# atenpas/agile_grasp

Hardware: AMD Instinct MI355X
Metric: grasp hypotheses/sec on 300k-pt cloud @2000 samples (higher is better)
Workload: dtype f64

## Files before the change

### agile_grasp_amd/csrc/taubin.hip

```cpp
#include "agh_internal.h"

#include <cstring>
#include <utility>

#include "taubin_eigen.h"

namespace agh
{

constexpr int kSortBins = 256;
constexpr int kChunk = 56;

template <int CAP>
__device__ __forceinline__ void taubin_moments_sample(const int s, GridView gv, const float* __restrict__ xyz, int64_t stride,
  const int32_t* __restrict__ samples, int S, float r2f, double rpad, int first_class, double* __restrict__ sums,
  int32_t* __restrict__ nt, int32_t* __restrict__ status, float4* __restrict__ nbr, int64_t nbr_stride, int debug_stop,
  int n_points, int32_t* __restrict__ zero_flags, int32_t* __restrict__ scloud, long long* __restrict__ dbg,
  int32_t* __restrict__ ovf_out)
{
#ifdef AGH_DEBUG_HOOKS
#define AGH_MSTAMP(i) do { if (dbg && threadIdx.x == 0) dbg[(int64_t) blockIdx.x * 8 + (i)] = wall_clock64(); } while (0)
  long long mt_prod = 0, mt_cons = 0, mt_wait = 0, mt_last = 0;
#define AGH_MLAP(acc) do { if (dbg) { const long long now_ = wall_clock64(); acc += now_ - mt_last; mt_last = now_; } } while (0)
#else
#define AGH_MSTAMP(i) do { } while (0)
#define AGH_MLAP(acc) do { } while (0)
#endif
  AGH_MSTAMP(0);
  constexpr int kSortBytes = CAP * 8 + CAP * 2 + (kSortBins + 1) * 4 + kSortBins * 4;
  constexpr int kTS = kChunk + 2;
  constexpr int kTermBytes = kNumSums * kTS * 8;
  constexpr int kScratch = ((kSortBytes > kTermBytes ? kSortBytes : kTermBytes) + 15) & ~15;
  __shared__ float4 stage[CAP];
  __shared__ unsigned short slot[CAP];
  __shared__ __attribute__((aligned(16))) unsigned char scratch[kScratch];
  __shared__ RowTable rt;
  __shared__ int count;
  __shared__ int wsum[4];
  unsigned long long* key = reinterpret_cast<unsigned long long*>(scratch);
  unsigned short* perm = reinterpret_cast<unsigned short*>(scratch + CAP * 8);
  int* hist = reinterpret_cast<int*>(scratch + CAP * 8 + CAP * 2);
  int* fillc = hist + (kSortBins + 1);
  double* termbuf = reinterpret_cast<double*>(scratch);

  const int tid = threadIdx.x, lane = tid & 63, wave = tid >> 6;
  if (zero_flags && blockIdx.x == 0 && tid < 8)
    zero_flags[tid] = 0;
  if (!first_class && status[s] != kStatusOverflow)
    return;
  const int n_pts = n_points >= 0 ? n_points : gv.cloud_off[gv.n_clouds];
  if (samples[s] < 0 || samples[s] >= n_pts)
  {
    if (threadIdx.x == 0)
    {
      status[s] = samples[s] == kSampleSkip ? kStatusSkipped : kStatusBadIndex;
      nt[s] = 0;
    }
    return;
  }
  const float* qp = xyz + (int64_t) samples[s] * stride;
  const float qx = qp[0], qy = qp[1], qz = qp[2];
  {
    const int cloud = cloud_of_point(gv, samples[s]);
    gv = grid_of_cloud(gv, cloud);
    if (first_class && tid == 0)
      scloud[s] = cloud;
  }
  if (!(isfinite(qx) && isfinite(qy) && isfinite(qz)))
  {
    if (tid == 0)
    {
      status[s] = kStatusOk;
      nt[s] = 0;
    }
    return;
  }
  if (tid == 0)
    count = 0;
  for (int k = tid; k < kSortBins; k += 256)
  {
    hist[k] = 0;
    fillc[k] = 0;
  }
  build_rows(gv, qx, qy, qz, rpad, rt);
  if (rt.bad)
  {
    if (tid == 0)
    {
      status[s] = kStatusRows;
      nt[s] = 0;
    }
    return;
  }
  AGH_MSTAMP(1);
  const float binscale = (float) kSortBins / r2f;
  {
    FlatRows flat;
    flat.init(rt, lane);
    const int nseg = flat.segments();
    auto seg_load = [&](int j, int& r0, float4& p0, float4& p1, bool& h0, bool& h1) {
      int a0, a1;
      flat.locate(j, r0, lane, a0, a1, h0, h1);
      p0 = gv.sorted[h0 ? a0 : 0];
      p1 = gv.sorted[h1 ? a1 : 0];
    };
    auto take2 = [&](const float4& p0, bool h0, const float4& p1, bool h1) {
      const float d0 = flann_d2(qx, qy, qz, p0.x, p0.y, p0.z), d1 = flann_d2(qx, qy, qz, p1.x, p1.y, p1.z);
      const bool s0 = h0 & (d0 < r2f), s1 = h1 & (d1 < r2f);
      const unsigned long long m0 = __ballot(s0), m1 = __ballot(s1);
      if (m0 | m1)
      {
        const int c0 = __popcll(m0);
        int base = 0;
        if (lane == 0)
          base = atomicAdd(&count, c0 + __popcll(m1));
        base = __builtin_amdgcn_readfirstlane(base);
        const unsigned long long below = (1ull << lane) - 1ull;
        const int k0 = base + __popcll(m0 & below), k1 = base + c0 + __popcll(m1 & below);
        if (s0 && k0 < CAP)
        {
          stage[k0] = p0;
          key[k0] = ((unsigned long long) __float_as_uint(d0) << 32) | (unsigned long long) __float_as_uint(p0.w);
          atomicAdd(&hist[min(kSortBins - 1, (int) (d0 * binscale))], 1);
        }
        if (s1 && k1 < CAP)
        {
          stage[k1] = p1;
          key[k1] = ((unsigned long long) __float_as_uint(d1) << 32) | (unsigned long long) __float_as_uint(p1.w);
          atomicAdd(&hist[min(kSortBins - 1, (int) (d1 * binscale))], 1);
        }
      }
    };
    int cur_j = wave, r0 = 0;
    float4 p0, p1;
    bool h0, h1;
    seg_load(cur_j, r0, p0, p1, h0, h1);
    while (cur_j < nseg)
    {
      float4 q0, q1;
      bool g0, g1;
      seg_load(cur_j + 4, r0, q0, q1, g0, g1);
      take2(p0, h0, p1, h1);
      cur_j += 4;
      p0 = q0;
      p1 = q1;
      h0 = g0;
      h1 = g1;
    }
  }
  __syncthreads();
  const int n = count;
  if (n > CAP)
  {
    if (tid == 0)
    {
      status[s] = kStatusOverflow;
      nt[s] = n;
      if (ovf_out)
        ovf_out[1 + atomicAdd(&ovf_out[0], 1)] = s;
    }
    return;
  }
  AGH_MSTAMP(2);
  if (debug_stop == 1)
    return;
  {
    const int lane_ = tid & 63, w_ = tid >> 6;
    const int v = hist[tid];
    const int inc = wave_incl_scan_i32(v);
    if (lane_ == 63)
      wsum[w_] = inc;
    __syncthreads();
    int base = 0;
    for (int k = 0; k < w_; k++)
      base += wsum[k];
    hist[tid] = base + inc - v;
    if (tid == 0)
      hist[kSortBins] = n;
    __syncthreads();
  }
  {
    constexpr int kPerThread = CAP <= 1152 ? (CAP + 255) / 256 : 1;
    for (int k0 = tid; k0 < n; k0 += 256 * kPerThread)
    {
      int bb[kPerThread], pos[kPerThread];
#pragma unroll
      for (int u = 0; u < kPerThread; u++)
      {
        const int k = k0 + 256 * u;
        const float d2 = __uint_as_float((unsigned) (key[k < n ? k : k0] >> 32));
        bb[u] = min(kSortBins - 1, (int) (d2 * binscale));
      }
#pragma unroll
      for (int u = 0; u < kPerThread; u++)
        pos[u] = (k0 + 256 * u < n) ? hist[bb[u]] + atomicAdd(&fillc[bb[u]], 1) : 0;
#pragma unroll
      for (int u = 0; u < kPerThread; u++)
        if (k0 + 256 * u < n)
          perm[pos[u]] = (unsigned short) (k0 + 256 * u);
    }
  }
  __syncthreads();
  for (int g = tid; g < n; g += 256)
  {
    const int k = perm[g];
    const unsigned long long mine = key[k];
    const float d2 = __uint_as_float((unsigned) (mine >> 32));
    const int b = min(kSortBins - 1, (int) (d2 * binscale));
    const int bs = hist[b], be = hist[b + 1];
    int rank = bs;
    for (int g2 = bs; g2 < be; g2 += 4)
    {
      unsigned short pk[4];
#pragma unroll
      for (int u = 0; u < 4; u++)
        pk[u] = perm[min(g2 + u, be - 1)];
      unsigned long long kk[4];
#pragma unroll
      for (int u = 0; u < 4; u++)
        kk[u] = key[pk[u]];
#pragma unroll
      for (int u = 0; u < 4; u++)
        rank += (g2 + u < be && kk[u] < mine) ? 1 : 0;
    }
    slot[rank] = (unsigned short) k;
  }
  __syncthreads();
  if (debug_stop == 2)
    return;
  AGH_MSTAMP(3);
  {
    constexpr int kPerThread = CAP <= 1152 ? (CAP + 255) / 256 : 1;
    for (int i0 = tid; i0 < n; i0 += 256 * kPerThread)
    {
      unsigned short sl[kPerThread];
#pragma unroll
      for (int u = 0; u < kPerThread; u++)
        sl[u] = slot[min(i0 + 256 * u, n > 0 ? n - 1 : 0)];
      float4 pv[kPerThread];
#pragma unroll
      for (int u = 0; u < kPerThread; u++)
        pv[u] = stage[sl[u]];
#pragma unroll
      for (int u = 0; u < kPerThread; u++)
        if (i0 + 256 * u < n)
          nbr[(int64_t) s * nbr_stride + i0 + 256 * u] = pv[u];
    }
  }
  double acc = 0.0;
#ifdef AGH_DEBUG_HOOKS
  mt_last = wall_clock64();
#endif
  const int n_last = n > 0 ? n - 1 : 0;
  float4 p_next = stage[slot[min(lane, n_last)]];
  for (int c0 = 0; c0 < n; c0 += kChunk)
  {
    const int rows = min(kChunk, n - c0);
    const float4 p = p_next;
    p_next = stage[slot[min(c0 + kChunk + lane, n_last)]];
    if (lane < rows && wave < 2)
    {
      const double x = (double) p.x, y = (double) p.y, z = (double) p.z;
      const double x2 = x * x, y2 = y * y, z2 = z * z;
      const double xy = x * y, yz = y * z, xz = x * z;
      double* t = &termbuf[lane];
      if (wave == 0)
      {
        t[0 * kTS] = x2 * x2;
        t[1 * kTS] = x2 * y2;
        t[2 * kTS] = x2 * z2;
        t[3 * kTS] = x2 * xy;
        t[4 * kTS] = x2 * yz;
        t[5 * kTS] = x2 * xz;
        t[6 * kTS] = x2 * x;
        t[7 * kTS] = x2 * y;
        t[8 * kTS] = x2 * z;
        t[9 * kTS] = x2;
        t[10 * kTS] = y2 * y2;
        t[11 * kTS] = y2 * z2;
        t[12 * kTS] = y2 * xy;
        t[13 * kTS] = y2 * yz;
        t[14 * kTS] = y2 * xz;
        t[15 * kTS] = y2 * x;
        t[16 * kTS] = y2 * y;
        t[17 * kTS] = y2 * z;
        t[18 * kTS] = y2;
      }
      else
      {
        t[19 * kTS] = z2 * z2;
        t[20 * kTS] = z2 * xy;
        t[21 * kTS] = z2 * yz;
        t[22 * kTS] = z2 * xz;
        t[23 * kTS] = z2 * x;
        t[24 * kTS] = z2 * y;
        t[25 * kTS] = z2 * z;
        t[26 * kTS] = z2;
        t[27 * kTS] = x * yz;
        t[28 * kTS] = xy;
        t[29 * kTS] = yz;
        t[30 * kTS] = xz;
        t[31 * kTS] = x;
        t[32 * kTS] = y;
        t[33 * kTS] = z;
        t[34 * kTS] = x2 + y2;
        t[35 * kTS] = y2 + z2;
        t[36 * kTS] = x2 + z2;
      }
    }
    __syncthreads();
    AGH_MLAP(mt_prod);
    if (wave == 0 && lane < kNumSums && rows == kChunk)
    {
      double2 va[kChunk / 2];
#pragma unroll
      for (int u = 0; u < kChunk / 2; u++)
        va[u] = reinterpret_cast<const double2*>(termbuf + lane * kTS)[u];
#pragma unroll
      for (int u = 0; u < kChunk / 2; u++)
      {
        acc += va[u].x;
        acc += va[u].y;
      }
    }
    else if (wave == 0 && lane < kNumSums)
    {
      int k = 0;
      for (; k + 8 <= rows; k += 8)
      {
        double v_[8];
#pragma unroll
        for (int u = 0; u < 8; u++)
          v_[u] = termbuf[lane * kTS + k + u];
#pragma unroll
        for (int u = 0; u < 8; u++)
          acc += v_[u];
      }
      for (; k < rows; k++)
        acc += termbuf[lane * kTS + k];
    }
#ifdef AGH_DEBUG_HOOKS
    if (dbg && acc == 1.2345e300)
      mt_cons++;
#endif
    AGH_MLAP(mt_cons);
    __syncthreads();
    AGH_MLAP(mt_wait);
  }
  if (wave == 0 && lane < kNumSums)
    sums[(int64_t) s * kSumStride + lane] = acc;
  if (tid == 0)
  {
    nt[s] = n;
    status[s] = kStatusOk;
  }
  AGH_MSTAMP(4);
#ifdef AGH_DEBUG_HOOKS
  if (dbg && threadIdx.x == 0)
  {
    dbg[(int64_t) blockIdx.x * 8 + 5] = mt_prod;
    dbg[(int64_t) blockIdx.x * 8 + 6] = mt_cons;
    dbg[(int64_t) blockIdx.x * 8 + 7] = mt_wait;
  }
#endif
#undef AGH_MSTAMP
#undef AGH_MLAP
}

template <int CAP>
__global__ __launch_bounds__(256, CAP <= 1152 ? 4 : 1) void k_taubin_moments(GridView gv, const float* __restrict__ xyz, int64_t stride,
  const int32_t* __restrict__ samples, int S, float r2f, double rpad, int first_class, double* __restrict__ sums,
  int32_t* __restrict__ nt, int32_t* __restrict__ status, float4* __restrict__ nbr, int64_t nbr_stride, int debug_stop,
  int n_points, int32_t* __restrict__ zero_flags, int32_t* __restrict__ scloud, long long* __restrict__ dbg,
  int32_t* __restrict__ ovf_out, const int32_t* __restrict__ ovf_list)
{
  if constexpr (CAP == 4096)
  {
    const int n_items = ovf_list ? min(ovf_list[0], S) : S;
    for (int it = blockIdx.x; it < n_items; it += gridDim.x)
    {
      taubin_moments_sample<CAP>(ovf_list ? ovf_list[1 + it] : it, gv, xyz, stride, samples, S, r2f, rpad, first_class, sums, nt, status,
        nbr, nbr_stride, debug_stop, n_points, zero_flags, scloud, dbg, ovf_out);
      if (it + (int) gridDim.x < n_items)
        __syncthreads();
    }
  }
  else
    taubin_moments_sample<CAP>((int) blockIdx.x, gv, xyz, stride, samples, S, r2f, rpad, first_class, sums, nt, status, nbr, nbr_stride,
      debug_stop, n_points, zero_flags, scloud, dbg, ovf_out);
}

__global__ __launch_bounds__(256) void k_taubin_moments_huge(GridView gv, const float* __restrict__ xyz, int64_t stride,
  const int32_t* __restrict__ samples, int S, float r2f, double rpad, double* __restrict__ sums, int32_t* __restrict__ nt,
  int32_t* __restrict__ status, float4* __restrict__ nbr, int64_t nbr_stride, float4* __restrict__ pool_stage,
  unsigned long long* __restrict__ pool_key, float4* __restrict__ pool_sorted, long long* __restrict__ huge_base,
  unsigned long long* __restrict__ pool_count)
{
  constexpr int kTS = kChunk + 2;
  constexpr int kKeyTile = 2048;
  __shared__ __attribute__((aligned(16))) double termbuf[kNumSums * kTS];
  __shared__ unsigned long long ktile[kKeyTile];
  __shared__ RowTable rt;
  __shared__ int count, n_s;
  __shared__ long long base_s;
  const int s = blockIdx.x;
  const int tid = threadIdx.x, lane = tid & 63, wave = tid >> 6;
  if (tid == 0)
    huge_base[s] = -1;
  if (status[s] != kStatusOverflow)
    return;
  if (tid == 0)
    count = 0;
  const float* qp = xyz + (int64_t) samples[s] * stride;
  const float qx = qp[0], qy = qp[1], qz = qp[2];
  gv = grid_of_cloud(gv, cloud_of_point(gv, samples[s]));
  build_rows(gv, qx, qy, qz, rpad, rt);
  if (rt.bad)
    return;
  {
    int mine = 0;
    for (int j = tid; j < rt.total; j += 256)
    {
      const float4 p = gv.sorted[row_lookup(rt, j)];
      mine += flann_d2(qx, qy, qz, p.x, p.y, p.z) < r2f ? 1 : 0;
    }
    mine = wave_allsum_i32(mine);
    if (lane == 0 && mine)
      atomicAdd(&count, mine);
  }
  __syncthreads();
  if (tid == 0)
  {
    const int n0 = count;
    n_s = n0;
    const unsigned long long b0 = atomicAdd(pool_count, (unsigned long long) n0);
    base_s = b0 + (unsigned long long) n0 <= (unsigned long long) kHugeEntries ? (long long) b0 : -1;
    count = 0;
  }
  __syncthreads();
  const int n = n_s;
  const long long base = base_s;
  if (base < 0)
  {
    if (tid == 0)
      nt[s] = n;
    return;
  }
  float4* stage = pool_stage + base;
  unsigned long long* key = pool_key + base;
  for (int j = tid; j < rt.total; j += 256)
  {
    const float4 p = gv.sorted[row_lookup(rt, j)];
    const float d2 = flann_d2(qx, qy, qz, p.x, p.y, p.z);
    if (d2 < r2f)
    {
      const int k = atomicAdd(&count, 1);
      stage[k] = p;
      key[k] = ((unsigned long long) __float_as_uint(d2) << 32) | (unsigned long long) __float_as_uint(p.w);
    }
  }
  __threadfence();
  __syncthreads();
  const bool in_pool = n > nbr_stride;
  float4* const list_w = in_pool ? pool_sorted + base : nbr + (int64_t) s * nbr_stride;
  if (tid == 0)
    huge_base[s] = in_pool ? base : -1;
  for (int g0 = 0; g0 < n; g0 += 256 * 8)
  {
    constexpr int kPer = 8;
    unsigned long long mine[kPer];
    int rank[kPer];
#pragma unroll
    for (int u = 0; u < kPer; u++)
    {
      const int g = g0 + tid + 256 * u;
      mine[u] = g < n ? key[g] : ~0ull;
      rank[u] = 0;
    }
    for (int t0 = 0; t0 < n; t0 += kKeyTile)
    {
      const int tn = min(kKeyTile, n - t0);
      __syncthreads();
      for (int k = tid; k < tn; k += 256)
        ktile[k] = key[t0 + k];
      __syncthreads();
      for (int k = 0; k < tn; k++)
      {
        const unsigned long long kk = ktile[k];
#pragma unroll
        for (int u = 0; u < kPer; u++)
          rank[u] += kk < mine[u] ? 1 : 0;
      }
    }
#pragma unroll
    for (int u = 0; u < kPer; u++)
    {
      const int g = g0 + tid + 256 * u;
      if (g < n)
        list_w[rank[u]] = stage[g];
    }
  }
  __threadfence();
  __syncthreads();
  const float4* list = list_w;
  double acc = 0.0;
  for (int c0 = 0; c0 < n; c0 += kChunk)
  {
    const int rows = min(kChunk, n - c0);
    if (lane < rows && wave < 2)
    {
      const float4 p = list[c0 + lane];
      const double x = (double) p.x, y = (double) p.y, z = (double) p.z;
      const double x2 = x * x, y2 = y * y, z2 = z * z;
      const double xy = x * y, yz = y * z, xz = x * z;
      double* t = &termbuf[lane];
      if (wave == 0)
      {
        t[0 * kTS] = x2 * x2;
        t[1 * kTS] = x2 * y2;
        t[2 * kTS] = x2 * z2;
        t[3 * kTS] = x2 * xy;
        t[4 * kTS] = x2 * yz;
        t[5 * kTS] = x2 * xz;
        t[6 * kTS] = x2 * x;
        t[7 * kTS] = x2 * y;
        t[8 * kTS] = x2 * z;
        t[9 * kTS] = x2;
        t[10 * kTS] = y2 * y2;
        t[11 * kTS] = y2 * z2;
        t[12 * kTS] = y2 * xy;
        t[13 * kTS] = y2 * yz;
        t[14 * kTS] = y2 * xz;
        t[15 * kTS] = y2 * x;
        t[16 * kTS] = y2 * y;
        t[17 * kTS] = y2 * z;
        t[18 * kTS] = y2;
      }
      else
      {
        t[19 * kTS] = z2 * z2;
        t[20 * kTS] = z2 * xy;
        t[21 * kTS] = z2 * yz;
        t[22 * kTS] = z2 * xz;
        t[23 * kTS] = z2 * x;
        t[24 * kTS] = z2 * y;
        t[25 * kTS] = z2 * z;
        t[26 * kTS] = z2;
        t[27 * kTS] = x * yz;
        t[28 * kTS] = xy;
        t[29 * kTS] = yz;
        t[30 * kTS] = xz;
        t[31 * kTS] = x;
        t[32 * kTS] = y;
        t[33 * kTS] = z;
        t[34 * kTS] = x2 + y2;
        t[35 * kTS] = y2 + z2;
        t[36 * kTS] = x2 + z2;
      }
    }
    __syncthreads();
    if (wave == 0 && lane < kNumSums)
      for (int k = 0; k < rows; k++)
        acc += termbuf[lane * kTS + k];
    __syncthreads();
  }
  if (wave == 0 && lane < kNumSums)
    sums[(int64_t) s * kSumStride + lane] = acc;
  if (tid == 0)
  {
    nt[s] = n;
    status[s] = kStatusOk;
  }
}

constexpr int kOrderBins = 2048;
constexpr int kOrderMaxSamples = 4096;
__device__ __forceinline__ int order_bin(int w) { return kOrderBins - 1 - min(w >> 4, kOrderBins - 1); }

__device__ void sample_order_block(const int* __restrict__ weight, int S, int* __restrict__ order, int* hist, int* wave_tot)
{
  constexpr int kPer = 16, kT = 256;
  const int tid = threadIdx.x, lane = tid & 63, wave = tid >> 6;
  for (int b = tid; b < kOrderBins; b += kT)
    hist[b] = 0;
  __syncthreads();
  for (int base = 0; base < S; base += kT * kPer)
  {
    int bin[kPer];
#pragma unroll
    for (int u = 0; u < kPer; u++)
    {
      const int s = base + u * kT + tid;
      bin[u] = s < S ? order_bin(weight[s]) : -1;
    }
#pragma unroll
    for (int u = 0; u < kPer; u++)
      if (bin[u] >= 0)
        atomicAdd(&hist[bin[u]], 1);
  }
  __syncthreads();
  constexpr int per = kOrderBins / kT;
  int loc = 0;
  for (int k = 0; k < per; k++)
    loc += hist[tid * per + k];
  int incl = loc;
  incl = wave_incl_scan_i32(incl);
  if (lane == 63)
    wave_tot[wave] = incl;
  __syncthreads();
  int run = incl - loc;
  for (int w = 0; w < wave; w++)
    run += wave_tot[w];
  for (int k = 0; k < per; k++)
  {
    const int c = hist[tid * per + k];
    hist[tid * per + k] = run;
    run += c;
  }
  __syncthreads();
  for (int base = 0; base < S; base += kT * kPer)
  {
    int bin[kPer], pos[kPer];
#pragma unroll
    for (int u = 0; u < kPer; u++)
    {
      const int s = base + u * kT + tid;
      bin[u] = s < S ? order_bin(weight[s]) : -1;
    }
#pragma unroll
    for (int u = 0; u < kPer; u++)
      pos[u] = bin[u] >= 0 ? atomicAdd(&hist[bin[u]], 1) : 0;
#pragma unroll
    for (int u = 0; u < kPer; u++)
      if (bin[u] >= 0)
        order[pos[u]] = base + u * kT + tid;
  }
}

constexpr int kSweepBlock = 32, kSweepBlocksMax = 1024;
__device__ void sweep_order_block(const int* __restrict__ weight, int S, int* __restrict__ order2, int* bw )
{
  const int B = (S + kSweepBlock - 1) / kSweepBlock;
  if (B > kSweepBlocksMax)
    return;
  const int tid = threadIdx.x;
  __syncthreads();
  for (int b = tid; b < B; b += 256)
  {
    int w = 0;
    const int i0 = b * kSweepBlock, i1 = min(S, i0 + kSweepBlock);
    for (int i = i0; i < i1; i++)
      w += weight[i];
    bw[b] = w;
  }
  __syncthreads();
  const int last_size = S - (B - 1) * kSweepBlock;
  int rank_last = 0;
  for (int q = 0; q < B - 1; q++)
    rank_last += bw[q] >= bw[B - 1] ? 1 : 0;
  for (int b = tid; b < B; b += 256)
  {
    const int wb = bw[b];
    int rank = 0;
// ... 1055 lines not shown
```

Baseline: 4.238 million.

## Double-buffer Taubin term tiles so producers overlap the reducing wave

Splits the moment loop into a software pipeline. Waves 1 and 2 produce the per-point term tile for the next chunk into one buffer while wave 0 reduces the previous chunk from another buffer. The second buffer reuses the now-dead stage array, which removes one of the two block barriers per chunk when it is large enough. Producers read points from the already-written global neighbour list rather than through the slot/stage indirection. The cost is an extra pipeline iteration and reliance on global reads and on stage being free after the copy-out.

```diff
diff --git a/agile_grasp_amd/csrc/taubin.hip b/agile_grasp_amd/csrc/taubin.hip
--- a/agile_grasp_amd/csrc/taubin.hip
+++ b/agile_grasp_amd/csrc/taubin.hip
@@ -31,6 +31,7 @@
   constexpr int kTS = kChunk + 2;
   constexpr int kTermBytes = kNumSums * kTS * 8;
   constexpr int kScratch = ((kSortBytes > kTermBytes ? kSortBytes : kTermBytes) + 15) & ~15;
+  constexpr bool kOverlap = CAP * 16 >= kTermBytes;
   __shared__ float4 stage[CAP];
   __shared__ unsigned short slot[CAP];
   __shared__ __attribute__((aligned(16))) unsigned char scratch[kScratch];
@@ -247,75 +248,104 @@
           nbr[(int64_t) s * nbr_stride + i0 + 256 * u] = pv[u];
     }
   }
+  double* tw = termbuf;
+  const double* tr = termbuf;
+  const float4* const list = nbr + (int64_t) s * nbr_stride;
+  const int n_last = n > 0 ? n - 1 : 0;
+  typedef float float3v __attribute__((ext_vector_type(3)));
+  float3v p_next = *reinterpret_cast<const float3v*>(&stage[slot[min(lane, n_last)]]);
+  if constexpr (kOverlap)
+  {
+    static_assert(sizeof(stage) >= kTermBytes, "the second term tile lies over stage");
+    __syncthreads();
+    tw = reinterpret_cast<double*>(stage);
+  }
   double acc = 0.0;
 #ifdef AGH_DEBUG_HOOKS
   mt_last = wall_clock64();
 #endif
-  const int n_last = n > 0 ? n - 1 : 0;
-  float4 p_next = stage[slot[min(lane, n_last)]];
-  for (int c0 = 0; c0 < n; c0 += kChunk)
-  {
+  for (int c0 = kOverlap ? -kChunk : 0; c0 < n; c0 += kChunk)
+  {
+    const int cp = kOverlap ? c0 + kChunk : c0;
+    const int rows_p = min(kChunk, n - cp);
+    if constexpr (kOverlap)
+    {
+      const double* const t_ = tr;
+      tr = tw;
+      tw = const_cast<double*>(t_);
+    }
+    if (wave == 1 || wave == 2)
+    {
+      asm volatile("" : "+v"(p_next));
+      double x = (double) p_next.x, y = (double) p_next.y, z = (double) p_next.z;
+      asm volatile("" : "+v"(x), "+v"(y), "+v"(z) : : "memory");
+      if constexpr (kOverlap)
+        p_next = *reinterpret_cast<const float3v*>(&list[min(cp + kChunk + lane, n_last)]);
+      else
+        p_next = *reinterpret_cast<const float3v*>(&stage[slot[min(cp + kChunk + lane, n_last)]]);
+      if (lane < rows_p)
+      {
+        const double x2 = x * x, y2 = y * y, z2 = z * z;
+        const double xy = x * y, yz = y * z, xz = x * z;
+        double* t = &tw[lane];
+        if (wave == 1)
+        {
+          t[0 * kTS] = x2 * x2;
+          t[1 * kTS] = x2 * y2;
+          t[2 * kTS] = x2 * z2;
+          t[3 * kTS] = x2 * xy;
+          t[4 * kTS] = x2 * yz;
+          t[5 * kTS] = x2 * xz;
+          t[6 * kTS] = x2 * x;
+          t[7 * kTS] = x2 * y;
+          t[8 * kTS] = x2 * z;
+          t[9 * kTS] = x2;
+          t[10 * kTS] = y2 * y2;
+          t[11 * kTS] = y2 * z2;
+          t[12 * kTS] = y2 * xy;
+          t[13 * kTS] = y2 * yz;
+          t[14 * kTS] = y2 * xz;
+          t[15 * kTS] = y2 * x;
+          t[16 * kTS] = y2 * y;
+          t[17 * kTS] = y2 * z;
+          t[18 * kTS] = y2;
+        }
+        else
+        {
+          t[19 * kTS] = z2 * z2;
+          t[20 * kTS] = z2 * xy;
+          t[21 * kTS] = z2 * yz;
+          t[22 * kTS] = z2 * xz;
+          t[23 * kTS] = z2 * x;
+          t[24 * kTS] = z2 * y;
+          t[25 * kTS] = z2 * z;
+          t[26 * kTS] = z2;
+          t[27 * kTS] = x * yz;
+          t[28 * kTS] = xy;
+          t[29 * kTS] = yz;
+          t[30 * kTS] = xz;
+          t[31 * kTS] = x;
+          t[32 * kTS] = y;
+          t[33 * kTS] = z;
+          t[34 * kTS] = x2 + y2;
+          t[35 * kTS] = y2 + z2;
+          t[36 * kTS] = x2 + z2;
+        }
+      }
+      AGH_MLAP(mt_prod);
+    }
+    if constexpr (!kOverlap)
+    {
+      __syncthreads();
+      AGH_MLAP(mt_wait);
+    }
     const int rows = min(kChunk, n - c0);
-    const float4 p = p_next;
-    p_next = stage[slot[min(c0 + kChunk + lane, n_last)]];
-    if (lane < rows && wave < 2)
-    {
-      const double x = (double) p.x, y = (double) p.y, z = (double) p.z;
-      const double x2 = x * x, y2 = y * y, z2 = z * z;
-      const double xy = x * y, yz = y * z, xz = x * z;
-      double* t = &termbuf[lane];
-      if (wave == 0)
-      {
-        t[0 * kTS] = x2 * x2;
-        t[1 * kTS] = x2 * y2;
-        t[2 * kTS] = x2 * z2;
-        t[3 * kTS] = x2 * xy;
-        t[4 * kTS] = x2 * yz;
-        t[5 * kTS] = x2 * xz;
-        t[6 * kTS] = x2 * x;
-        t[7 * kTS] = x2 * y;
-        t[8 * kTS] = x2 * z;
-        t[9 * kTS] = x2;
-        t[10 * kTS] = y2 * y2;
-        t[11 * kTS] = y2 * z2;
-        t[12 * kTS] = y2 * xy;
-        t[13 * kTS] = y2 * yz;
-        t[14 * kTS] = y2 * xz;
-        t[15 * kTS] = y2 * x;
-        t[16 * kTS] = y2 * y;
-        t[17 * kTS] = y2 * z;
-        t[18 * kTS] = y2;
-      }
-      else
-      {
-        t[19 * kTS] = z2 * z2;
-        t[20 * kTS] = z2 * xy;
-        t[21 * kTS] = z2 * yz;
-        t[22 * kTS] = z2 * xz;
-        t[23 * kTS] = z2 * x;
-        t[24 * kTS] = z2 * y;
-        t[25 * kTS] = z2 * z;
-        t[26 * kTS] = z2;
-        t[27 * kTS] = x * yz;
-        t[28 * kTS] = xy;
-        t[29 * kTS] = yz;
-        t[30 * kTS] = xz;
-        t[31 * kTS] = x;
-        t[32 * kTS] = y;
-        t[33 * kTS] = z;
-        t[34 * kTS] = x2 + y2;
-        t[35 * kTS] = y2 + z2;
-        t[36 * kTS] = x2 + z2;
-      }
-    }
-    __syncthreads();
-    AGH_MLAP(mt_prod);
-    if (wave == 0 && lane < kNumSums && rows == kChunk)
+    if (wave == 0 && lane < kNumSums && c0 >= 0 && rows == kChunk)
     {
       double2 va[kChunk / 2];
 #pragma unroll
       for (int u = 0; u < kChunk / 2; u++)
-        va[u] = reinterpret_cast<const double2*>(termbuf + lane * kTS)[u];
+        va[u] = reinterpret_cast<const double2*>(tr + lane * kTS)[u];
 #pragma unroll
       for (int u = 0; u < kChunk / 2; u++)
       {
@@ -323,7 +353,7 @@
         acc += va[u].y;
       }
     }
-    else if (wave == 0 && lane < kNumSums)
+    else if (wave == 0 && lane < kNumSums && c0 >= 0)
     {
       int k = 0;
       for (; k + 8 <= rows; k += 8)
@@ -331,19 +361,20 @@
         double v_[8];
 #pragma unroll
         for (int u = 0; u < 8; u++)
-          v_[u] = termbuf[lane * kTS + k + u];
+          v_[u] = tr[lane * kTS + k + u];
 #pragma unroll
         for (int u = 0; u < 8; u++)
           acc += v_[u];
       }
       for (; k < rows; k++)
-        acc += termbuf[lane * kTS + k];
+        acc += tr[lane * kTS + k];
     }
 #ifdef AGH_DEBUG_HOOKS
     if (dbg && acc == 1.2345e300)
       mt_cons++;
+    if (wave == 0)
+      AGH_MLAP(mt_cons);
 #endif
-    AGH_MLAP(mt_cons);
     __syncthreads();
     AGH_MLAP(mt_wait);
   }
@@ -356,9 +387,10 @@
   }
   AGH_MSTAMP(4);
 #ifdef AGH_DEBUG_HOOKS
+  if (dbg && threadIdx.x == 64)
+    dbg[(int64_t) blockIdx.x * 8 + 5] = mt_prod;
   if (dbg && threadIdx.x == 0)
   {
-    dbg[(int64_t) blockIdx.x * 8 + 5] = mt_prod;
     dbg[(int64_t) blockIdx.x * 8 + 6] = mt_cons;
     dbg[(int64_t) blockIdx.x * 8 + 7] = mt_wait;
   }
```

Result: faster. 4.334 million, median of 6 (+2.3%).
